# voitta-ai/voitta-rag

Measured on AMD Instinct MI355X. Metric: chunks indexed/sec + p50 top-10 query latency @1M-chunk corpus, 1/8 MI355X, higher is better.
Workload: dtype f16 (f16 MFMA operands, f32 accumulate; softmax, LayerNorm statistics and pooling in f32; the residual stream between layers is stored as f16 (LayerNorm is applied inside the GEMM epilogues from f32 row sums); measured |1-cos| = 1.5e-6 vs the f64 oracle on THIS code path at this scale — 2300 sequenc

## Files before the change

voitta_rag_amd/csrc/prefilter.hip:

```cpp


#include "engine_internal.h"
#include "topk_device.h"

#include <algorithm>
#include <cmath>
#include <vector>

namespace vr {

using f32x4 = __attribute__((ext_vector_type(4))) float;
using f16x8 = __attribute__((ext_vector_type(8))) _Float16;
using half_t = _Float16;

constexpr int kK16 = 32;


__global__ __launch_bounds__(256) void shadow_rows_kernel(const float* __restrict__ corpus, int64_t first_row,
                                                          int64_t n, int dim, int kblocks,
                                                          half_t* __restrict__ corpus16,
                                                          float* __restrict__ row_err) {
  const int lane = threadIdx.x & 63;
  const int64_t row = first_row + static_cast<int64_t>(blockIdx.x) * 4 + (threadIdx.x >> 6);
  if (row >= first_row + n) return;
  const int64_t tile = row / kTileRows;
  const int r = static_cast<int>(row % kTileRows);
  const int kb16n = dim / kK16;
  float e2 = 0.0f;
  for (int k = lane; k < dim; k += 64) {
    const int kb = k / kTileK, kk = k % kTileK;
    const float x = corpus[((tile * kblocks + kb) * 64 + tile_pos(kk % 4, r)) * 4 + kk / 4];
    const float xc = fminf(fmaxf(x, -65504.0f), 65504.0f);
    const half_t h = static_cast<half_t>(xc);
    const float d = x - static_cast<float>(h);
    e2 += d * d;
    const int kb16 = k / kK16, g = (k % kK16) / 8, j = k % 8;
    corpus16[((tile * kb16n + kb16) * 64 + g * 16 + r) * 8 + j] = h;
  }
#pragma unroll
  for (int off = 32; off >= 1; off >>= 1) e2 += __shfl_xor(e2, off);
  if (lane == 0) row_err[row] = sqrtf(e2) * 1.001f + 1.0e-12f;
}

using i32x4 = __attribute__((ext_vector_type(4))) int;
constexpr int kK8 = 64;

__global__ __launch_bounds__(256) void shadow_rows8_kernel(const float* __restrict__ corpus, int64_t first_row,
                                                           int64_t n, int dim, int kblocks,
                                                           int8_t* __restrict__ corpus8,
                                                           float* __restrict__ row_scale,
                                                           float* __restrict__ row_err,
                                                           const float* __restrict__ centre, float centre_norm) {
  const int lane = threadIdx.x & 63;
  const int64_t row = first_row + static_cast<int64_t>(blockIdx.x) * 4 + (threadIdx.x >> 6);
  if (row >= first_row + n) return;
  const int64_t tile = row / kTileRows;
  const int r = static_cast<int>(row % kTileRows);
  const int kb8n = dim / kK8;
  auto at = [&](int k) {
    const int kb = k / kTileK, kk = k % kTileK;
    const float x = corpus[((tile * kblocks + kb) * 64 + tile_pos(kk % 4, r)) * 4 + kk / 4];
    return centre ? x - centre[k] : x;
  };
  float mx = 0.0f;
  for (int k = lane; k < dim; k += 64) mx = fmaxf(mx, fabsf(at(k)));
#pragma unroll
  for (int off = 32; off >= 1; off >>= 1) mx = fmaxf(mx, __shfl_xor(mx, off));
  const bool finite = mx <= 3.0e38f;
  const float s = finite ? mx / 127.0f : 0.0f;
  const float inv = finite && mx > 0.0f ? 127.0f / mx : 0.0f;
  float e2 = 0.0f;
  for (int k = lane; k < dim; k += 64) {
    const float x = at(k);
    const float t = fminf(fmaxf(rintf(x * inv), -127.0f), 127.0f);
    const float d = x - s * t;
    e2 += d * d;
    corpus8[((tile * kb8n + k / kK8) * 64 + ((k % kK8) / 16) * 16 + r) * 16 + k % 16] = static_cast<int8_t>(t);
  }
#pragma unroll
  for (int off = 32; off >= 1; off >>= 1) e2 += __shfl_xor(e2, off);
  if (lane == 0) {
    row_scale[row] = s;
    row_err[row] = finite ? sqrtf(e2) * 1.001f + 2.4e-7f * mx * sqrtf(static_cast<float>(dim)) + 1.0e-12f +
                                (centre ? 1.2e-7f * (1.001f + centre_norm) : 0.0f)
                          : __builtin_inff();
  }
}

int prefilter_store_rows(vr_engine* e, int64_t n, int64_t first_row) {
  if (!e->prefilter || n <= 0) return 0;
  if (e->prefilter8)
    hipLaunchKernelGGL(shadow_rows8_kernel, dim3(static_cast<unsigned>((n + 3) / 4)), dim3(256), 0, e->stream,
                       e->corpus.p, first_row, n, e->dim, e->kblocks, reinterpret_cast<int8_t*>(e->corpus16.p),
                       e->row_scale.p, e->row_err.p, e->centre_rows > 0 ? e->centre.p : static_cast<const float*>(nullptr),
                       e->centre_norm);
  else
    hipLaunchKernelGGL(shadow_rows_kernel, dim3(static_cast<unsigned>((n + 3) / 4)), dim3(256), 0, e->stream,
                       e->corpus.p, first_row, n, e->dim, e->kblocks, reinterpret_cast<half_t*>(e->corpus16.p),
                       e->row_err.p);
  VR_HIP(hipGetLastError());
  return 0;
}

__global__ __launch_bounds__(256) void column_sum_kernel(const float* __restrict__ corpus, int64_t n_rows, int kblocks,
                                                         float* __restrict__ sum) {
  const int64_t tile0 = static_cast<int64_t>(blockIdx.x) * 64;
  const int64_t n_tiles = (n_rows + kTileRows - 1) / kTileRows;
  for (int p = threadIdx.x; p < kblocks * 256; p += 256) {
    const int kb = p >> 8, pos = (p >> 2) & 63, c = p & 3;
    const int r = pos >> 2;
    float acc = 0.0f;
    for (int64_t t = tile0; t < min(tile0 + 64, n_tiles); ++t)
      if (t * kTileRows + r < n_rows) acc += corpus[(t * kblocks + kb) * 256 + p - (kb << 8)];
    atomicAdd(sum + kb * kTileK + (pos & 3) + 4 * c, acc);
  }
}

__global__ void centre_from_sum_kernel(const float* __restrict__ sum, int dim, float inv_n, float* __restrict__ centre) {
  const int k = blockIdx.x * blockDim.x + threadIdx.x;
  if (k < dim) centre[k] = sum[k] * inv_n;
}

constexpr int64_t kCentreMinRows = 1024;

int prefilter_recentre(vr_engine* e) {
  if (!e->prefilter || !e->prefilter8 || e->n_rows <= 0) return 0;
  const bool centring = !(getenv("VR_PREFILTER_CENTRE") && atoi(getenv("VR_PREFILTER_CENTRE")) == 0);
  if (!centring) e->centre_rows = 0;
  e->centre_checked_rows = e->n_rows;
  if (centring && e->n_rows >= kCentreMinRows) {
    static_assert(kTileK == 16, "column_sum_kernel decodes the [k/16][lane][4] image");
    VR_TRY(e->centre.grow(e->dim, 0, e->stream));
    VR_TRY(e->centre_sum.grow(e->dim, 0, e->stream));
    VR_HIP(hipMemsetAsync(e->centre_sum.p, 0, sizeof(float) * static_cast<size_t>(e->dim), e->stream));
    const int64_t n_tiles = (e->n_rows + kTileRows - 1) / kTileRows;
    hipLaunchKernelGGL(column_sum_kernel, dim3(static_cast<unsigned>((n_tiles + 63) / 64)), dim3(256), 0, e->stream,
                       e->corpus.p, e->n_rows, e->kblocks, e->centre_sum.p);
    hipLaunchKernelGGL(centre_from_sum_kernel, dim3(static_cast<unsigned>((e->dim + 255) / 256)), dim3(256), 0, e->stream,
                       e->centre_sum.p, e->dim, 1.0f / static_cast<float>(e->n_rows), e->centre.p);
    VR_HIP(hipGetLastError());
    std::vector<float> host(static_cast<size_t>(e->dim));
    VR_HIP(hipMemcpyAsync(host.data(), e->centre.p, sizeof(float) * host.size(), hipMemcpyDeviceToHost, e->stream));
    VR_HIP(hipStreamSynchronize(e->stream));
    double n2 = 0.0;
    bool finite = true;
    for (float v : host) {
      n2 += static_cast<double>(v) * v;
      finite = finite && std::isfinite(v);
    }
    if (!centring) {
      e->centre_norm = 0.0f;
      e->centre_rows = 0;
    } else if (finite) {
      e->centre_norm = static_cast<float>(std::sqrt(n2) * 1.000001 + 1e-30);
      e->centre_rows = e->n_rows;
    } else {
      e->centre_norm = 0.0f;
      e->centre_rows = 0;
    }
  }
  return prefilter_store_rows(e, e->n_rows, 0);
}


constexpr int kScan16Waves = 8;

__global__ __launch_bounds__(kScan16Waves * 64) void prefilter_scan_kernel(
    const uint4* __restrict__ corpus16, const float* __restrict__ q_img, const float* __restrict__ row_err,
    const uint8_t* __restrict__ mask, int64_t n_tiles, int kb16n, int dim, int k, float* __restrict__ upper,
    uint64_t* __restrict__ cand, int32_t* __restrict__ counter) {
  extern __shared__ uint4 q_lds[];
  __shared__ float red[kScan16Waves];
  uint64_t* lists = reinterpret_cast<uint64_t*>(q_lds + 2 * kb16n * 64);
  if (blockIdx.x == 0 && threadIdx.x == 0) counter[0] = counter[1] = 0;
  for (int i = threadIdx.x; i < 2 * kb16n * 64; i += kScan16Waves * 64) q_lds[i] = make_uint4(0, 0, 0, 0);
  for (int i = threadIdx.x; i < kScan16Waves * kListLen; i += kScan16Waves * 64) lists[i] = 0ull;
  __syncthreads();
  float n2 = 0.0f;
  {
    half_t* qh = reinterpret_cast<half_t*>(q_lds);
    half_t* ql = qh + kb16n * 512;
    for (int kk = threadIdx.x; kk < dim; kk += kScan16Waves * 64) {
      const int kb = kk / kTileK, kr = kk % kTileK;
      const float q = q_img[(kb * 64 + (kr % 4) * 16 + 0) * 4 + kr / 4];
      n2 += q * q;
      const float qc = fminf(fmaxf(q, -65504.0f), 65504.0f);
      const half_t hi = static_cast<half_t>(qc);
      const half_t lo = static_cast<half_t>(qc - static_cast<float>(hi));
      const int at = ((kk / kK16) * 64 + ((kk % kK16) / 8) * 16 + 0) * 8 + kk % 8;
      qh[at] = hi;
      ql[at] = lo;
    }
  }
#pragma unroll
  for (int off = 32; off >= 1; off >>= 1) n2 += __shfl_xor(n2, off);
  if ((threadIdx.x & 63) == 0) red[threadIdx.x >> 6] = n2;
  __syncthreads();
  float qn2 = 0.0f;
#pragma unroll
  for (int w = 0; w < kScan16Waves; ++w) qn2 += red[w];
  const float qn = sqrtf(qn2) * 1.0001f + 1.0e-12f;
  const float c_fixed = 1.001f * (4.8e-7f * qn + 6.0e-8f * sqrtf(static_cast<float>(dim))) +
                        static_cast<float>(dim) * 5.0e-7f * fmaxf(qn, 1.0f);
  const int lane = threadIdx.x & 63;
  const int wave = threadIdx.x >> 6;
  uint64_t* mine = lists + wave * kListLen;
  const bool active = (lane & 15) == 0;
  const int64_t wave_stride = static_cast<int64_t>(gridDim.x) * kScan16Waves;
  for (int64_t tile = static_cast<int64_t>(blockIdx.x) * kScan16Waves + wave; tile < n_tiles; tile += wave_stride) {
    const uint4* src = corpus16 + tile * kb16n * 64 + lane;
    const int64_t row0 = tile * kTileRows + (lane >> 4) * 4;
    uchar4 m = make_uchar4(0, 0, 0, 0);
    float4 e4 = make_float4(0.f, 0.f, 0.f, 0.f);
    if (active) {
      m = *reinterpret_cast<const uchar4*>(mask + row0);
      e4 = *reinterpret_cast<const float4*>(row_err + row0);
    }
    f32x4 acc = {0.0f, 0.0f, 0.0f, 0.0f};
    int kb = 0;
    for (; kb + 8 <= kb16n; kb += 8) {
      uint4 a[8];
#pragma unroll
      for (int u = 0; u < 8; ++u) a[u] = src[(kb + u) * 64];
#pragma unroll
      for (int u = 0; u < 8; ++u) {
        const uint4 bh = q_lds[(kb + u) * 64 + lane];
        const uint4 bl = q_lds[(kb16n + kb + u) * 64 + lane];
        acc = __builtin_amdgcn_mfma_f32_16x16x32_f16(*reinterpret_cast<const f16x8*>(&a[u]),
                                                     *reinterpret_cast<const f16x8*>(&bh), acc, 0, 0, 0);
        acc = __builtin_amdgcn_mfma_f32_16x16x32_f16(*reinterpret_cast<const f16x8*>(&a[u]),
                                                     *reinterpret_cast<const f16x8*>(&bl), acc, 0, 0, 0);
      }
    }
    for (; kb < kb16n; ++kb) {
      const uint4 a = src[kb * 64];
      const uint4 bh = q_lds[kb * 64 + lane];
      const uint4 bl = q_lds[(kb16n + kb) * 64 + lane];
      acc = __builtin_amdgcn_mfma_f32_16x16x32_f16(*reinterpret_cast<const f16x8*>(&a),
                                                   *reinterpret_cast<const f16x8*>(&bh), acc, 0, 0, 0);
      acc = __builtin_amdgcn_mfma_f32_16x16x32_f16(*reinterpret_cast<const f16x8*>(&a),
                                                   *reinterpret_cast<const f16x8*>(&bl), acc, 0, 0, 0);
    }
    uint64_t key[4] = {0, 0, 0, 0};
    if (active) {
      const unsigned char mm[4] = {m.x, m.y, m.z, m.w};
      const float ee[4] = {e4.x, e4.y, e4.z, e4.w};
      float up[4];
#pragma unroll
      for (int r = 0; r < 4; ++r) {
        const float a = acc[r];
        const float err = ee[r] * qn + c_fixed + 2.0e-7f * fabsf(a);
        up[r] = mm[r] ? a + err : -__builtin_inff();
        key[r] = mm[r] ? topk_make_key(a - err, row0 + r) : 0ull;
      }
      *reinterpret_cast<float4*>(upper + row0) = make_float4(up[0], up[1], up[2], up[3]);
    }
    const uint64_t thr = active ? mine[k - 1] : ~0ull;
    if (__ballot(key[0] > thr || key[1] > thr || key[2] > thr || key[3] > thr)) {
#pragma unroll
      for (int r = 0; r < 4; ++r) wave_offer(mine, k, key[r], 0, active, lane);
    }
  }
  block_merge_lists(lists, kListLen, kScan16Waves, wave, lane);
  if (wave == 0) cand[static_cast<int64_t>(blockIdx.x) * kListLen + lane] = lists[lane];
}


__global__ __launch_bounds__(kScan16Waves * 64) void prefilter_scan8_kernel(
    const uint4* __restrict__ corpus8, const float* __restrict__ q_img, const float* __restrict__ row_err,
    const float* __restrict__ row_scale, const uint8_t* __restrict__ mask, int64_t n_tiles, int kb8n, int dim, int k,
    float* __restrict__ upper, uint64_t* __restrict__ cand, int32_t* __restrict__ counter, float centre_norm) {
  extern __shared__ uint4 q_lds[];
  __shared__ float red[3][kScan16Waves];
  uint64_t* lists = reinterpret_cast<uint64_t*>(q_lds + 2 * kb8n * 64);
  if (blockIdx.x == 0 && threadIdx.x == 0) counter[0] = counter[1] = 0;
  for (int i = threadIdx.x; i < 2 * kb8n * 64; i += kScan16Waves * 64) q_lds[i] = make_uint4(0, 0, 0, 0);
  for (int i = threadIdx.x; i < kScan16Waves * kListLen; i += kScan16Waves * 64) lists[i] = 0ull;
  auto q_at = [&](int kk) {
    const int kb = kk / kTileK, kr = kk % kTileK;
    return q_img[(kb * 64 + (kr % 4) * 16 + 0) * 4 + kr / 4];
  };
  float mx = 0.0f, n2 = 0.0f;
  for (int kk = threadIdx.x; kk < dim; kk += kScan16Waves * 64) {
    const float q = q_at(kk);
    mx = fmaxf(mx, fabsf(q));
    n2 += q * q;
  }
#pragma unroll
  for (int off = 32; off >= 1; off >>= 1) {
    mx = fmaxf(mx, __shfl_xor(mx, off));
    n2 += __shfl_xor(n2, off);
  }
  if ((threadIdx.x & 63) == 0) {
    red[0][threadIdx.x >> 6] = mx;
    red[1][threadIdx.x >> 6] = n2;
  }
  __syncthreads();
  float t = 0.0f, qn2 = 0.0f;
#pragma unroll
  for (int w = 0; w < kScan16Waves; ++w) {
    t = fmaxf(t, red[0][w]);
    qn2 += red[1][w];
  }
  const bool q_ok = t > 0.0f && t <= 3.0e38f;
  const float a = q_ok ? t / 127.0f : 0.0f;
  const float inv_a = q_ok ? 127.0f / t : 0.0f;
  const float b = a / 254.0f;
  const float inv_b = a > 0.0f ? 254.0f / a : 0.0f;
  float rho2 = 0.0f;
  {
    int8_t* qa = reinterpret_cast<int8_t*>(q_lds);
    int8_t* qb = qa + kb8n * 1024;
    for (int kk = threadIdx.x; kk < dim; kk += kScan16Waves * 64) {
      const float q = q_at(kk);
      const float ta = fminf(fmaxf(rintf(q * inv_a), -127.0f), 127.0f);
      const float r = q - a * ta;
      const float tb = fminf(fmaxf(rintf(r * inv_b), -127.0f), 127.0f);
      const float rho = r - b * tb;
      rho2 += rho * rho;
      const int at = ((kk / kK8) * 64 + ((kk % kK8) / 16) * 16 + 0) * 16 + kk % 16;
      qa[at] = static_cast<int8_t>(ta);
      qb[at] = static_cast<int8_t>(tb);
    }
  }
#pragma unroll
  for (int off = 32; off >= 1; off >>= 1) rho2 += __shfl_xor(rho2, off);
  if ((threadIdx.x & 63) == 0) red[2][threadIdx.x >> 6] = rho2;
  __syncthreads();
  float rho2_all = 0.0f;
#pragma unroll
  for (int w = 0; w < kScan16Waves; ++w) rho2_all += red[2][w];
  const float qn = sqrtf(qn2) * 1.0001f + 1.0e-12f;
  const float rho_n = q_ok ? sqrtf(rho2_all) * 1.001f + 3.0e-7f * qn + 1.0e-12f : __builtin_inff();
  const float c_fixed = static_cast<float>(dim) * 5.0e-7f * fmaxf(qn, 1.0f) + 1.0e-7f * qn * sqrtf(static_cast<float>(dim)) +
                        centre_norm * rho_n;
  const int lane = threadIdx.x & 63;
  const int wave = threadIdx.x >> 6;
  uint64_t* mine = lists + wave * kListLen;
  const bool active = (lane & 15) == 0;
  const int64_t wave_stride = static_cast<int64_t>(gridDim.x) * kScan16Waves;
  for (int64_t tile = static_cast<int64_t>(blockIdx.x) * kScan16Waves + wave; tile < n_tiles; tile += wave_stride) {
    const uint4* src = corpus8 + tile * kb8n * 64 + lane;
    const int64_t row0 = tile * kTileRows + (lane >> 4) * 4;
    uchar4 m = make_uchar4(0, 0, 0, 0);
    float4 e4 = make_float4(0.f, 0.f, 0.f, 0.f), s4 = e4;
    if (active) {
      m = *reinterpret_cast<const uchar4*>(mask + row0);
      e4 = *reinterpret_cast<const float4*>(row_err + row0);
      s4 = *reinterpret_cast<const float4*>(row_scale + row0);
    }
    i32x4 acc_a = {0, 0, 0, 0}, acc_b = {0, 0, 0, 0};
    int kb = 0;
    for (; kb + 6 <= kb8n; kb += 6) {
      uint4 v[6];
#pragma unroll
      for (int u = 0; u < 6; ++u) v[u] = src[(kb + u) * 64];
#pragma unroll
      for (int u = 0; u < 6; ++u) {
        const uint4 ba = q_lds[(kb + u) * 64 + lane];
        const uint4 bb = q_lds[(kb8n + kb + u) * 64 + lane];
        acc_a = __builtin_amdgcn_mfma_i32_16x16x64_i8(*reinterpret_cast<const i32x4*>(&v[u]),
                                                      *reinterpret_cast<const i32x4*>(&ba), acc_a, 0, 0, 0);
        acc_b = __builtin_amdgcn_mfma_i32_16x16x64_i8(*reinterpret_cast<const i32x4*>(&v[u]),
                                                      *reinterpret_cast<const i32x4*>(&bb), acc_b, 0, 0, 0);
      }
    }
    for (; kb < kb8n; ++kb) {
      const uint4 v = src[kb * 64];
      const uint4 ba = q_lds[kb * 64 + lane];
      const uint4 bb = q_lds[(kb8n + kb) * 64 + lane];
      acc_a = __builtin_amdgcn_mfma_i32_16x16x64_i8(*reinterpret_cast<const i32x4*>(&v),
                                                    *reinterpret_cast<const i32x4*>(&ba), acc_a, 0, 0, 0);
      acc_b = __builtin_amdgcn_mfma_i32_16x16x64_i8(*reinterpret_cast<const i32x4*>(&v),
                                                    *reinterpret_cast<const i32x4*>(&bb), acc_b, 0, 0, 0);
    }
    uint64_t key[4] = {0, 0, 0, 0};
    if (active) {
      const unsigned char mm[4] = {m.x, m.y, m.z, m.w};
      const float ee[4] = {e4.x, e4.y, e4.z, e4.w};
      const float ss[4] = {s4.x, s4.y, s4.z, s4.w};
      float up[4];
#pragma unroll
      for (int r = 0; r < 4; ++r) {
        const float fa = a * static_cast<float>(acc_a[r]);
        const float fb = b * static_cast<float>(acc_b[r]);
        const float score = ss[r] * (fa + fb);
        const float err = ee[r] * qn + (1.001f + ee[r]) * rho_n + c_fixed + 2.0e-6f * ss[r] * (fabsf(fa) + fabsf(fb));
        up[r] = mm[r] ? score + err : -__builtin_inff();
        key[r] = mm[r] ? topk_make_key(score - err, row0 + r) : 0ull;
      }
      *reinterpret_cast<float4*>(upper + row0) = make_float4(up[0], up[1], up[2], up[3]);
    }
    const uint64_t thr = active ? mine[k - 1] : ~0ull;
    if (__ballot(key[0] > thr || key[1] > thr || key[2] > thr || key[3] > thr)) {
#pragma unroll
      for (int r = 0; r < 4; ++r) wave_offer(mine, k, key[r], 0, active, lane);
    }
  }
  block_merge_lists(lists, kListLen, kScan16Waves, wave, lane);
  if (wave == 0) cand[static_cast<int64_t>(blockIdx.x) * kListLen + lane] = lists[lane];
}


__device__ __forceinline__ float key_score(uint64_t key) {
  const uint32_t hi = static_cast<uint32_t>(key >> 32);
  const uint32_t u = (hi & 0x80000000u) ? (hi ^ 0x80000000u) : ~hi;
  return __uint_as_float(u);
}

__global__ __launch_bounds__(256) void collect_candidates_kernel(const float* __restrict__ upper, int64_t n,
                                                                 const uint64_t* __restrict__ lower_keys, int k,
                                                                 int32_t* __restrict__ tiles,
                                                                 int32_t* __restrict__ masks, int32_t* counter) {
  const uint64_t kth = lower_keys[k - 1];
  const float thr = kth ? key_score(kth) : -3.0e38f;
  const int lane = threadIdx.x & 63;
  const int64_t base = (static_cast<int64_t>(blockIdx.x) * blockDim.x + threadIdx.x) * 4;
  float4 u = make_float4(-__builtin_inff(), -__builtin_inff(), -__builtin_inff(), -__builtin_inff());
  if (base < n) u = *reinterpret_cast<const float4*>(upper + base);
  const float uu[4] = {u.x, u.y, u.z, u.w};
  int m = 0;
#pragma unroll
  for (int c = 0; c < 4; ++c)
    if (base + c < n && uu[c] >= thr) m |= 1 << c;
  if (__ballot(m != 0) == 0) return;
  int m16 = m << (4 * (lane & 3));
  m16 |= __shfl_xor(m16, 1);
  m16 |= __shfl_xor(m16, 2);
  const bool take = (lane & 3) == 0 && m16 != 0;
  const uint64_t takers = __ballot(take);
  int rows_here = take ? __popc(m16) : 0;
#pragma unroll
  for (int off = 32; off >= 1; off >>= 1) rows_here += __shfl_xor(rows_here, off);
  const int leader = __builtin_ctzll(takers);
  int slot0 = 0;
  if (lane == leader) {
    slot0 = atomicAdd(counter, __popcll(takers));
    atomicAdd(counter + 1, rows_here);
  }
  slot0 = __shfl(slot0, leader);
  const int slot = slot0 + __popcll(takers & ((1ull << lane) - 1ull));
  if (take && slot < kMaxCandTiles) {
    tiles[slot] = static_cast<int32_t>(base / kTileRows);
    masks[slot] = m16;
  }
}


constexpr int kRescoreThreads = 1024;
constexpr int kRescoreBlocks = 128;
constexpr int kRescoreChunk = 64;

__global__ __launch_bounds__(kRescoreThreads) void rescore_kernel(const float4* __restrict__ corpus,
                                                                  const float4* __restrict__ q_img, int kblocks,
                                                                  const int32_t* __restrict__ tiles,
                                                                  const int32_t* __restrict__ masks,
                                                                  const int32_t* __restrict__ counter, int k,
                                                                  uint64_t* __restrict__ lists_out,
                                                                  int32_t* __restrict__ out_count) {
  extern __shared__ float4 stage[];
  __shared__ uint64_t best[kListLen];
  const int chunk = min(kblocks, kRescoreChunk);
  const bool q_resident = kblocks <= kRescoreChunk;
  const int n_tiles = counter[0];
  const int count = min(n_tiles, kMaxCandTiles);
  const int lane = threadIdx.x & 63;
  const int wave = threadIdx.x >> 6;
  if (blockIdx.x == 0 && threadIdx.x == 0) *out_count = n_tiles > kMaxCandTiles ? 0x7fffffff : counter[1];
  if (threadIdx.x < kListLen) best[threadIdx.x] = 0ull;
  bool q_staged = !q_resident;
  const bool active = (lane & 15) == 0;
  for (int c = blockIdx.x; c < count; c += gridDim.x) {
    const int64_t tile = tiles[c];
    const int mask = masks[c];
    f32x4 acc = {0.0f, 0.0f, 0.0f, 0.0f};
    for (int kb0 = 0; kb0 < kblocks; kb0 += chunk) {
      const int nkb = min(chunk, kblocks - kb0);
      const float4* a_src = corpus + (tile * kblocks + kb0) * 64;
      const float4* b_src = q_img + kb0 * 64;
      __syncthreads();
#pragma unroll 4
      for (int i = threadIdx.x; i < nkb * 64; i += kRescoreThreads) {
        stage[i] = a_src[i];
        if (!q_staged || !q_resident) stage[chunk * 64 + i] = b_src[i];
      }
      q_staged = true;
      __syncthreads();
      if (wave == 0) {
#pragma unroll 4
        for (int kb = 0; kb < nkb; ++kb) {
          const float4 a = stage[kb * 64 + tile_pos(lane >> 4, lane & 15)];
          const float4 b = stage[(chunk + kb) * 64 + lane];
          acc = __builtin_amdgcn_mfma_f32_16x16x4f32(a.x, b.x, acc, 0, 0, 0);
          acc = __builtin_amdgcn_mfma_f32_16x16x4f32(a.y, b.y, acc, 0, 0, 0);
          acc = __builtin_amdgcn_mfma_f32_16x16x4f32(a.z, b.z, acc, 0, 0, 0);
          acc = __builtin_amdgcn_mfma_f32_16x16x4f32(a.w, b.w, acc, 0, 0, 0);
        }
      }
    }
    if (wave == 0) {
      const int r0 = (lane >> 4) * 4;
#pragma unroll
      for (int r = 0; r < 4; ++r) {
        const uint64_t key = active && ((mask >> (r0 + r)) & 1) ? topk_make_key(acc[r], tile * kTileRows + r0 + r) : 0ull;
        wave_offer(best, k, key, 0, active, lane);
      }
    }
  }
  __syncthreads();
  if (wave == 0) lists_out[static_cast<int64_t>(blockIdx.x) * kListLen + lane] = best[lane];
}

bool prefilter_usable(vr_engine* e, int nq, int k) {
  return e->prefilter && nq == 1 && k <= kFusedMaxK && e->n_rows >= 4096;
}

int prefilter_search(vr_engine* e, int k, const uint8_t* mask_dev, uint64_t* out_keys_dev, int32_t* out_count_dev) {
  const int kb16n = e->dim / kK16;
  const int64_t n_tiles = (e->n_rows + kTileRows - 1) / kTileRows;
  VR_TRY(e->upper.grow(e->cap_rows, 0, e->stream));
  VR_TRY(e->cand_rows.grow(2 * kMaxCandTiles + 16, 0, e->stream));
  int64_t blocks = std::min<int64_t>((n_tiles + kScan16Waves - 1) / kScan16Waves, kScanBlocks);
  VR_TRY(e->cand_a.grow(std::max<int64_t>(blocks, kRescoreBlocks) * kListLen, 0, e->stream));
  VR_TRY(e->cand_b.grow(kListLen, 0, e->stream));
  int32_t* counter = e->cand_rows.p + 2 * kMaxCandTiles;
  hipStream_t s = e->stream;
  if (e->prefilter8) {
    const int kb8n = e->dim / kK8;
    const size_t lds = static_cast<size_t>(2) * kb8n * 1024 + kScan16Waves * kListLen * sizeof(uint64_t);
    if (lds > 64 * 1024)
      VR_HIP(hipFuncSetAttribute(reinterpret_cast<const void*>(prefilter_scan8_kernel),
                                 hipFuncAttributeMaxDynamicSharedMemorySize, static_cast<int>(lds)));
    prof_begin(e, VR_PROF_DENSE_SCAN, static_cast<double>(e->n_rows) * (e->dim * 1.0 + 4.0 + 4.0 + 1.0 + 4.0));
    hipLaunchKernelGGL(prefilter_scan8_kernel, dim3(static_cast<unsigned>(blocks)), dim3(kScan16Waves * 64), lds, s,
                       reinterpret_cast<const uint4*>(e->corpus16.p), e->q_tiled.p, e->row_err.p, e->row_scale.p,
                       mask_dev, n_tiles, kb8n, e->dim, k, e->upper.p, e->cand_a.p, counter,
                       e->centre_rows > 0 ? e->centre_norm : 0.0f);
    prof_end(e);
  } else {
    const size_t lds = static_cast<size_t>(2) * kb16n * 1024 + kScan16Waves * kListLen * sizeof(uint64_t);
    if (lds > 64 * 1024)
      VR_HIP(hipFuncSetAttribute(reinterpret_cast<const void*>(prefilter_scan_kernel),
                                 hipFuncAttributeMaxDynamicSharedMemorySize, static_cast<int>(lds)));
    prof_begin(e, VR_PROF_DENSE_SCAN, static_cast<double>(e->n_rows) * (e->dim * 2.0 + 4.0 + 1.0 + 4.0));
    hipLaunchKernelGGL(prefilter_scan_kernel, dim3(static_cast<unsigned>(blocks)), dim3(kScan16Waves * 64), lds, s,
                       reinterpret_cast<const uint4*>(e->corpus16.p), e->q_tiled.p, e->row_err.p, mask_dev, n_tiles,
                       kb16n, e->dim, k, e->upper.p, e->cand_a.p, counter);
    prof_end(e);
  }
  VR_TRY(topk_merge_lists(e, e->cand_a.p, static_cast<int>(blocks), 1, k, e->cand_b.p));
  const int64_t n4 = (e->n_rows + 3) / 4;
  int32_t* cand_tiles = e->cand_rows.p;
  int32_t* cand_masks = e->cand_rows.p + kMaxCandTiles;
  hipLaunchKernelGGL(collect_candidates_kernel, dim3(static_cast<unsigned>((n4 + 255) / 256)), dim3(256), 0, s,
                     e->upper.p, e->n_rows, e->cand_b.p, k, cand_tiles, cand_masks, counter);
  const size_t rescore_lds = static_cast<size_t>(2) * std::min(e->kblocks, kRescoreChunk) * 1024;
  if (rescore_lds > 64 * 1024)
    VR_HIP(hipFuncSetAttribute(reinterpret_cast<const void*>(rescore_kernel),
                               hipFuncAttributeMaxDynamicSharedMemorySize, static_cast<int>(rescore_lds)));
  hipLaunchKernelGGL(rescore_kernel, dim3(kRescoreBlocks), dim3(kRescoreThreads), rescore_lds, s,
                     reinterpret_cast<const float4*>(e->corpus.p),
                     reinterpret_cast<const float4*>(e->q_tiled.p), e->kblocks, cand_tiles, cand_masks, counter, k,
                     e->cand_a.p, out_count_dev);
  VR_TRY(topk_merge_lists(e, e->cand_a.p, kRescoreBlocks, 1, k, out_keys_dev));
  VR_HIP(hipGetLastError());
  return 0;
}

}
```

voitta_rag_amd/csrc/topk.hip:

```cpp

#include "engine_internal.h"
#include "topk_device.h"

namespace vr {

__device__ __forceinline__ uint64_t make_key(float s, int64_t row) {
  if (s == -__builtin_inff()) return 0ull;
  uint32_t u = __float_as_uint(s);
  u = (u & 0x80000000u) ? ~u : (u | 0x80000000u);
  return (static_cast<uint64_t>(u) << 32) | static_cast<uint32_t>(0xFFFFFFFFu - static_cast<uint32_t>(row));
}

template <int THREADS, int ITEMS>
__device__ __forceinline__ void block_extract_topk(uint64_t (&keys)[ITEMS], int k,
                                                   uint64_t* __restrict__ out) {
  constexpr int WAVES = THREADS / 64;
  __shared__ uint64_t wmax[2][WAVES];
  const int lane = threadIdx.x & 63;
  const int wave = threadIdx.x >> 6;

  uint64_t lmax = 0;
#pragma unroll
  for (int i = 0; i < ITEMS; ++i) lmax = keys[i] > lmax ? keys[i] : lmax;

  for (int r = 0; r < k; ++r) {
    uint64_t m = lmax;
#pragma unroll
    for (int off = 32; off >= 1; off >>= 1) {
      uint64_t o = __shfl_xor(m, off);
      m = o > m ? o : m;
    }
    if (lane == 0) wmax[r & 1][wave] = m;
    __syncthreads();
    uint64_t best = 0;
#pragma unroll
    for (int w = 0; w < WAVES; ++w) {
      uint64_t v = wmax[r & 1][w];
      best = v > best ? v : best;
    }
    if (threadIdx.x == 0) out[r] = best;
    if (best == 0) {
      for (int j = r + 1 + threadIdx.x; j < k; j += THREADS) out[j] = 0;
      break;
    }
    if (lmax == best) {
      lmax = 0;
#pragma unroll
      for (int i = 0; i < ITEMS; ++i) {
        if (keys[i] == best) keys[i] = 0;
        lmax = keys[i] > lmax ? keys[i] : lmax;
      }
    }
  }
}

template <int THREADS, int ITEMS>
__global__ __launch_bounds__(THREADS) void select_from_scores_kernel(
    const float* __restrict__ scores, int64_t stride, int64_t n, int k, uint64_t* __restrict__ out) {
  const int64_t seg = blockIdx.x;
  const int q = blockIdx.y;
  const int64_t base = seg * (THREADS * ITEMS);
  const float* s = scores + q * stride;
  uint64_t keys[ITEMS];
#pragma unroll
  for (int i = 0; i < ITEMS; ++i) {
    int64_t row = base + i * THREADS + threadIdx.x;
    keys[i] = row < n ? make_key(s[row], row) : 0ull;
  }
  block_extract_topk<THREADS, ITEMS>(keys, k, out + (static_cast<int64_t>(q) * gridDim.x + seg) * k);
}

template <int THREADS, int ITEMS>
__global__ __launch_bounds__(THREADS) void select_from_keys_kernel(const uint64_t* __restrict__ in,
                                                                   int64_t count, int k,
                                                                   uint64_t* __restrict__ out) {
  const int64_t seg = blockIdx.x;
  const int q = blockIdx.y;
  const int64_t base = seg * (THREADS * ITEMS);
  const uint64_t* s = in + q * count;
  uint64_t keys[ITEMS];
#pragma unroll
  for (int i = 0; i < ITEMS; ++i) {
    int64_t j = base + i * THREADS + threadIdx.x;
    keys[i] = j < count ? s[j] : 0ull;
  }
  block_extract_topk<THREADS, ITEMS>(keys, k, out + (static_cast<int64_t>(q) * gridDim.x + seg) * k);
}

template <int THREADS, int ITEMS>
__global__ __launch_bounds__(THREADS) void select_regions_kernel(const uint64_t* __restrict__ in, int n_reg, int cap,
                                                                 const int32_t* __restrict__ cnt,
                                                                 const uint64_t* __restrict__ spill, int spill_cap,
                                                                 const int32_t* __restrict__ spill_cnt, int k,
                                                                 uint64_t* __restrict__ out,
                                                                 int32_t* __restrict__ overflow,
                                                                 int32_t* __restrict__ total_out,
                                                                 int32_t* __restrict__ overflow_q) {
  __shared__ uint64_t gat[THREADS * ITEMS];
  __shared__ int n_gat;
  const int q = blockIdx.x;
  const int n_spill = spill_cnt ? spill_cnt[q] : 0;
  if (threadIdx.x == 0) n_gat = n_spill < spill_cap ? n_spill : spill_cap;
  __syncthreads();
  for (int j = threadIdx.x; j < n_spill && j < spill_cap; j += THREADS)
    if (j < THREADS * ITEMS) gat[j] = spill[static_cast<int64_t>(q) * spill_cap + j];
  const uint64_t* base = in + static_cast<int64_t>(q) * n_reg * cap;
  const int32_t* c = cnt + static_cast<int64_t>(q) * n_reg;
  for (int r = threadIdx.x; r < n_reg; r += THREADS) {
    const int have = c[r];
    if (have <= 0) continue;
    const int n = have < cap ? have : cap;
    const int at = atomicAdd(&n_gat, n);
    for (int j = 0; j < n; ++j)
      if (at + j < THREADS * ITEMS) gat[at + j] = base[static_cast<int64_t>(r) * cap + j];
  }
  __syncthreads();
  const int total = n_gat;
  if (threadIdx.x == 0) {
    if (total_out) atomicAdd(total_out, total);
    if (n_spill > spill_cap || total > THREADS * ITEMS) {
      *overflow = 1;
      if (overflow_q) overflow_q[q] = 1;
    }
  }
  uint64_t keys[ITEMS];
#pragma unroll
  for (int i = 0; i < ITEMS; ++i) {
    const int j = i * THREADS + static_cast<int>(threadIdx.x);
    keys[i] = j < total && j < THREADS * ITEMS ? gat[j] : 0ull;
  }
  block_extract_topk<THREADS, ITEMS>(keys, k, out + static_cast<int64_t>(q) * k);
}

int topk_select_regions(vr_engine* e, const uint64_t* cand, int n_reg, int cap, const int32_t* cnt, const uint64_t* spill,
                        int spill_cap, const int32_t* spill_cnt, int nq, int k, uint64_t* out, int32_t* overflow_mapped,
                        int32_t* total_dev, int32_t* overflow_q) {
  VR_CHECK(k >= 1 && k <= kMaxK && nq >= 1 && cap >= 1 && n_reg >= 1, "bad region-select shape");
  hipLaunchKernelGGL((select_regions_kernel<1024, 8>), dim3(static_cast<unsigned>(nq)), dim3(1024), 0, e->stream, cand, n_reg, cap,
                     cnt, spill, spill_cap, spill_cnt, k, out, overflow_mapped, total_dev, overflow_q);
  VR_HIP(hipGetLastError());
  return 0;
}


constexpr int kMergeThreads = 1024;
constexpr int kMergeWaves = kMergeThreads / 64;
constexpr int kMergeMaxLists = 512;
constexpr int kGatherCap = 2048;
constexpr int kGatherBatch = 16;

__global__ __launch_bounds__(kMergeThreads) void merge_lists_kernel(uint64_t* __restrict__ cand, int n_lists,
                                                                     int k, uint64_t* __restrict__ out) {
  __shared__ uint64_t gat[kGatherCap];
  __shared__ uint64_t wave_thr[kMergeWaves];
  __shared__ uint64_t heads[kMergeMaxLists];
  __shared__ uint64_t head_thr;
  __shared__ int gathered;
  const int lane = threadIdx.x & 63;
  const int wave = threadIdx.x >> 6;
  uint64_t* in = cand + static_cast<int64_t>(blockIdx.x) * n_lists * kListLen;
  uint64_t* dst = out + static_cast<int64_t>(blockIdx.x) * k;

  {
    uint64_t t = 0;
    if (static_cast<int>(threadIdx.x) < n_lists) {
      heads[threadIdx.x] = in[threadIdx.x * kListLen];
      t = in[threadIdx.x * kListLen + (k - 1)];
    }
#pragma unroll
    for (int off = 32; off >= 1; off >>= 1) {
      const uint64_t o = __shfl_xor(t, off);
      t = o > t ? o : t;
    }
    if (lane == 0) wave_thr[wave] = t;
    if (threadIdx.x == 0) {
      gathered = 0;
      head_thr = 0;
    }
    __syncthreads();
    if (static_cast<int>(threadIdx.x) < n_lists) {
      const uint64_t h = heads[threadIdx.x];
      int rank = 0;
      for (int j = 0; j < n_lists; ++j) rank += heads[j] > h;
      if (rank == k - 1 && h != 0) head_thr = h;
    }
    __syncthreads();
    uint64_t thr = head_thr;
#pragma unroll
    for (int w = 0; w < kMergeWaves; ++w) thr = wave_thr[w] > thr ? wave_thr[w] : thr;
    for (int l0 = wave; l0 < n_lists; l0 += kMergeWaves * kGatherBatch) {
      uint64_t keys[kGatherBatch];
#pragma unroll
      for (int u = 0; u < kGatherBatch; ++u) {
        const int l = min(l0 + u * kMergeWaves, n_lists - 1);
        keys[u] = in[l * kListLen + lane];
      }
#pragma unroll
      for (int u = 0; u < kGatherBatch; ++u) {
        const uint64_t key = keys[u];
        const bool take = l0 + u * kMergeWaves < n_lists && lane < k && key != 0 && key >= thr;
        const uint64_t m = __ballot(take);
        if (m) {
          int base = 0;
          if (lane == 0) base = atomicAdd(&gathered, __popcll(m));
          base = __builtin_amdgcn_readfirstlane(base);
          const int slot = base + __popcll(m & ((1ull << lane) - 1ull));
          if (take && slot < kGatherCap) gat[slot] = key;
        }
      }
    }
    __syncthreads();
    const int c = gathered;
    if (c <= kGatherCap) {
      for (int i = threadIdx.x; i < c; i += kMergeThreads) {
        const uint64_t key = gat[i];
        int rank = 0;
        for (int j = 0; j < c; ++j) rank += gat[j] > key;
        if (rank < k) dst[rank] = key;
      }
      for (int i = c + threadIdx.x; i < k; i += kMergeThreads) dst[i] = 0;
      return;
    }
  }
  int n = n_lists;
  while (n > 1) {
    const int pairs = (n + 1) / 2;
    for (int p0 = 0; p0 < pairs; p0 += kMergeWaves) {
      const int p = p0 + wave;
      uint64_t res = 0;
      if (p < pairs) {
        const uint64_t a = in[(2 * p) * kListLen + lane];
        const uint64_t b = (2 * p + 1 < n) ? in[(2 * p + 1) * kListLen + (63 - lane)] : 0ull;
        res = merge64(a, b, lane);
      }
      __syncthreads();
      if (p < pairs) in[p * kListLen + lane] = res;
    }
    __syncthreads();
    n = pairs;
  }
  if (wave == 0 && lane < k) dst[lane] = in[lane];
}

int topk_merge_lists(vr_engine* e, uint64_t* cand, int n_lists, int nq, int k, uint64_t* out) {
  VR_CHECK(k >= 1 && k <= kListLen && n_lists >= 1 && n_lists <= kMergeMaxLists, "bad merge shape");
  hipLaunchKernelGGL(merge_lists_kernel, dim3(static_cast<unsigned>(nq)), dim3(kMergeThreads), 0, e->stream,
                     cand, n_lists, k, out);
  VR_HIP(hipGetLastError());
  return 0;
}

constexpr int kPartsMax = 4096;

__global__ __launch_bounds__(256) void merge_parts_kernel(const uint64_t* __restrict__ parts, int n_parts, int n_lists,
                                                          int k, int64_t* __restrict__ gid, float* __restrict__ score,
                                                          int32_t* __restrict__ cnt) {
  __shared__ uint64_t keys[kPartsMax];
  __shared__ int total;
  const int l = blockIdx.x;
  const int n = n_parts * k;
  if (threadIdx.x == 0) total = 0;
  for (int i = threadIdx.x; i < n; i += 256) {
    const int p = i / k, j = i - p * k;
    keys[i] = parts[(static_cast<int64_t>(p) * n_lists + l) * k + j];
  }
  for (int j = threadIdx.x; j < k; j += 256) {
    gid[static_cast<int64_t>(l) * k + j] = -1;
    score[static_cast<int64_t>(l) * k + j] = 0.0f;
  }
  __syncthreads();
  int mine = 0;
  for (int i = threadIdx.x; i < n; i += 256) {
    const uint64_t key = keys[i];
    if (key == 0) continue;
    ++mine;
    int rank = 0;
    for (int o = 0; o < n; ++o) {
      const uint64_t ok = keys[o];
      rank += (ok > key) || (ok == key && o < i);
    }
    if (rank < k) {
      const uint32_t hi = static_cast<uint32_t>(key >> 32);
      const uint32_t u = (hi & 0x80000000u) ? (hi ^ 0x80000000u) : ~hi;
      const int64_t row = static_cast<int64_t>(0xFFFFFFFFu - static_cast<uint32_t>(key & 0xFFFFFFFFu));
      gid[static_cast<int64_t>(l) * k + rank] = row * n_parts + i / k;
      score[static_cast<int64_t>(l) * k + rank] = __uint_as_float(u);
    }
  }
  if (mine) atomicAdd(&total, mine);
  __syncthreads();
  if (threadIdx.x == 0) cnt[l] = total < k ? total : k;
}

int topk_merge_parts(vr_engine* e, const uint64_t* parts_dev, int n_parts, int n_lists, int k, int64_t* gid_dev,
                     float* score_dev, int32_t* cnt_dev) {
  VR_CHECK(n_parts >= 1 && n_lists >= 1 && k >= 1 && n_parts * k <= kPartsMax, "merge of %d parts x %d keys (at most %d keys per list)",
           n_parts, k, kPartsMax);
  hipLaunchKernelGGL(merge_parts_kernel, dim3(static_cast<unsigned>(n_lists)), dim3(256), 0, e->stream, parts_dev, n_parts,
                     n_lists, k, gid_dev, score_dev, cnt_dev);
  VR_HIP(hipGetLastError());
  return 0;
}

int topk_select(vr_engine* e, const float* scores, int64_t stride, int64_t n, int nq, int k,
                const uint64_t** out_keys) {
  VR_CHECK(k >= 1 && k <= kMaxK, "top-k of %d not in 1..%d", k, kMaxK);
  VR_CHECK(nq >= 1, "no queries");
  constexpr int T1 = 256, I1 = kTopkSeg / T1;
  constexpr int T2 = 1024, I2 = 16;
  int64_t nseg = (n + kTopkSeg - 1) / kTopkSeg;
  if (nseg < 1) nseg = 1;
  int64_t need = static_cast<int64_t>(nq) * nseg * k;
  VR_TRY(e->cand_a.grow(need, 0, e->stream));
  VR_TRY(e->cand_b.grow(need, 0, e->stream));
  hipLaunchKernelGGL((select_from_scores_kernel<T1, I1>), dim3(static_cast<unsigned>(nseg), nq),
                     dim3(T1), 0, e->stream, scores, stride, n, k, e->cand_a.p);
  uint64_t* cur = e->cand_a.p;
  uint64_t* nxt = e->cand_b.p;
  int64_t count = nseg * k;
  while (nseg > 1) {
    int64_t nseg2 = (count + T2 * I2 - 1) / (T2 * I2);
    hipLaunchKernelGGL((select_from_keys_kernel<T2, I2>), dim3(static_cast<unsigned>(nseg2), nq),
                       dim3(T2), 0, e->stream, cur, count, k, nxt);
    uint64_t* t = cur;
    cur = nxt;
    nxt = t;
    nseg = nseg2;
    count = nseg * k;
  }
  VR_HIP(hipGetLastError());
  *out_keys = cur;
  return 0;
}

}
```

voitta_rag_amd/csrc/topk_device.h:

```cpp
#pragma once

#include <hip/hip_runtime.h>

#include <cstdint>

namespace vr {

constexpr int kListLen = 64;

__device__ __forceinline__ uint64_t topk_make_key(float s, int64_t row) {
  if (s == -__builtin_inff()) return 0ull;
  uint32_t u = __float_as_uint(s);
  u = (u & 0x80000000u) ? ~u : (u | 0x80000000u);
  return (static_cast<uint64_t>(u) << 32) |
         static_cast<uint32_t>(0xFFFFFFFFu - static_cast<uint32_t>(row));
}

__device__ __forceinline__ uint64_t readlane_u64(uint64_t v, int src_lane) {
  uint32_t lo = __builtin_amdgcn_readlane(static_cast<uint32_t>(v), src_lane);
  uint32_t hi = __builtin_amdgcn_readlane(static_cast<uint32_t>(v >> 32), src_lane);
  return (static_cast<uint64_t>(hi) << 32) | lo;
}

__device__ __forceinline__ void wave_list_insert(uint64_t* list, int k, uint64_t key, int lane) {
  const uint64_t cur = list[lane];
  const uint64_t greater = __ballot(cur > key);
  const int pos = __popcll(greater);
  if (pos >= k) return;
  const uint64_t prev = __shfl_up(cur, 1);
  if (lane == pos) list[lane] = key;
  else if (lane > pos && lane < k) list[lane] = prev;
}

__device__ __forceinline__ void wave_offer(uint64_t* lists, int k, uint64_t key, int q_of_lane,
                                           bool active, int lane) {
  uint64_t thr = active ? lists[q_of_lane * kListLen + (k - 1)] : ~0ull;
  uint64_t pending = __ballot(active && key > thr);
  while (pending) {
    const int src = __builtin_ctzll(pending);
    const uint64_t kk = readlane_u64(key, src);
    const int qs = __builtin_amdgcn_readlane(q_of_lane, src);
    wave_list_insert(lists + qs * kListLen, k, kk, lane);
    pending &= pending - 1;
  }
}

__device__ __forceinline__ uint64_t merge64(uint64_t a, uint64_t b_reversed, int lane) {
  uint64_t v = a > b_reversed ? a : b_reversed;
#pragma unroll
  for (int d = 32; d >= 1; d >>= 1) {
    const uint64_t p = __shfl_xor(v, d);
    const bool keep_max = (lane & d) == 0;
    v = keep_max ? (v > p ? v : p) : (v < p ? v : p);
  }
  return v;
}

__device__ __forceinline__ void block_merge_lists(uint64_t* lists, int stride, int n_waves, int wave, int lane) {
  for (int s = 1; s < n_waves; s <<= 1) {
    __syncthreads();
    uint64_t merged = 0;
    const bool mine = (wave % (2 * s)) == 0;
    if (mine) merged = merge64(lists[wave * stride + lane], lists[(wave + s) * stride + (63 - lane)], lane);
    __syncthreads();
    if (mine) lists[wave * stride + lane] = merged;
  }
  __syncthreads();
}

}
```

Baseline: 46880.

## Fold list-merge threshold into candidate collection and rescore two tiles per block

```diff
diff --git a/voitta_rag_amd/csrc/prefilter.hip b/voitta_rag_amd/csrc/prefilter.hip
--- a/voitta_rag_amd/csrc/prefilter.hip
+++ b/voitta_rag_amd/csrc/prefilter.hip
@@ -408,11 +408,19 @@
   return __uint_as_float(u);
 }
 
-__global__ __launch_bounds__(256) void collect_candidates_kernel(const float* __restrict__ upper, int64_t n,
-                                                                 const uint64_t* __restrict__ lower_keys, int k,
-                                                                 int32_t* __restrict__ tiles,
-                                                                 int32_t* __restrict__ masks, int32_t* counter) {
-  const uint64_t kth = lower_keys[k - 1];
+constexpr int kCollectThreads = 1024;
+static_assert(kCollectThreads >= kScanBlocks, "lists_kth_lower_bound: a thread per list");
+
+__global__ __launch_bounds__(kCollectThreads) void collect_candidates_kernel(const float* __restrict__ upper, int64_t n,
+                                                                             const uint64_t* __restrict__ lists,
+                                                                             int n_lists, int k,
+                                                                             int32_t* __restrict__ tiles,
+                                                                             int32_t* __restrict__ masks,
+                                                                             int32_t* counter) {
+  __shared__ uint64_t heads[kScanBlocks];
+  __shared__ uint64_t wave_thr[kCollectThreads / 64];
+  __shared__ uint64_t head_thr;
+  const uint64_t kth = lists_kth_lower_bound(lists, n_lists, k, heads, wave_thr, &head_thr);
   const float thr = kth ? key_score(kth) : -3.0e38f;
   const int lane = threadIdx.x & 63;
   const int64_t base = (static_cast<int64_t>(blockIdx.x) * blockDim.x + threadIdx.x) * 4;
@@ -449,7 +457,9 @@
 
 constexpr int kRescoreThreads = 1024;
 constexpr int kRescoreBlocks = 128;
-constexpr int kRescoreChunk = 64;
+constexpr int kRescoreTiles = 2;
+constexpr int kRescoreChunk = 48;
+static_assert(kRescoreBlocks * kRescoreTiles <= kMaxCandTiles, "a block reads its first slots before it knows the tile count");
 
 __global__ __launch_bounds__(kRescoreThreads) void rescore_kernel(const float4* __restrict__ corpus,
                                                                   const float4* __restrict__ q_img, int kblocks,
@@ -459,38 +469,51 @@
                                                                   uint64_t* __restrict__ lists_out,
                                                                   int32_t* __restrict__ out_count) {
   extern __shared__ float4 stage[];
-  __shared__ uint64_t best[kListLen];
+  __shared__ uint64_t best[kRescoreTiles][kListLen];
   const int chunk = min(kblocks, kRescoreChunk);
-  const bool q_resident = kblocks <= kRescoreChunk;
+  float4* q_b = stage + kRescoreTiles * chunk * 64;
+  const int lane = threadIdx.x & 63;
+  const int wave = threadIdx.x >> 6;
+  const int blocks = static_cast<int>(gridDim.x);
+  int64_t tile0 = tiles[blockIdx.x], tile1 = tiles[blockIdx.x + blocks];
   const int n_tiles = counter[0];
   const int count = min(n_tiles, kMaxCandTiles);
-  const int lane = threadIdx.x & 63;
-  const int wave = threadIdx.x >> 6;
   if (blockIdx.x == 0 && threadIdx.x == 0) *out_count = n_tiles > kMaxCandTiles ? 0x7fffffff : counter[1];
-  if (threadIdx.x < kListLen) best[threadIdx.x] = 0ull;
-  bool q_staged = !q_resident;
+  if (threadIdx.x < kRescoreTiles * kListLen) (&best[0][0])[threadIdx.x] = 0ull;
+  for (int i = threadIdx.x; i < kblocks * 4; i += kRescoreThreads) q_b[i] = q_img[(i >> 2) * 64 + (i & 3) * 16];
   const bool active = (lane & 15) == 0;
-  for (int c = blockIdx.x; c < count; c += gridDim.x) {
-    const int64_t tile = tiles[c];
-    const int mask = masks[c];
+  for (int c0 = blockIdx.x; c0 < count; c0 += blocks * kRescoreTiles) {
+    const bool two = c0 + blocks < count;
+    if (c0 != static_cast<int>(blockIdx.x)) {
+      tile0 = tiles[c0];
+      tile1 = two ? tiles[c0 + blocks] : 0;
+    }
+    const int mine = c0 + wave * blocks;
+    const bool chains = wave < kRescoreTiles && mine < count;
+    const int mask = chains ? masks[mine] : 0;
     f32x4 acc = {0.0f, 0.0f, 0.0f, 0.0f};
     for (int kb0 = 0; kb0 < kblocks; kb0 += chunk) {
       const int nkb = min(chunk, kblocks - kb0);
-      const float4* a_src = corpus + (tile * kblocks + kb0) * 64;
-      const float4* b_src = q_img + kb0 * 64;
       __syncthreads();
-#pragma unroll 4
+      const float4* src0 = corpus + (tile0 * kblocks + kb0) * 64;
+      const float4* src1 = corpus + (tile1 * kblocks + kb0) * 64;
+#pragma unroll 2
       for (int i = threadIdx.x; i < nkb * 64; i += kRescoreThreads) {
-        stage[i] = a_src[i];
-        if (!q_staged || !q_resident) stage[chunk * 64 + i] = b_src[i];
-      }
-      q_staged = true;
+        const float4 v0 = src0[i];
+        if (two) {
+          const float4 v1 = src1[i];
+          stage[chunk * 64 + i] = v1;
+        }
+        stage[i] = v0;
+      }
       __syncthreads();
-      if (wave == 0) {
+      if (chains) {
+        const float4* a_lds = stage + wave * chunk * 64 + tile_pos(lane >> 4, lane & 15);
+        const float4* b_lds = q_b + kb0 * 4 + (lane >> 4);
 #pragma unroll 4
         for (int kb = 0; kb < nkb; ++kb) {
-          const float4 a = stage[kb * 64 + tile_pos(lane >> 4, lane & 15)];
-          const float4 b = stage[(chunk + kb) * 64 + lane];
+          const float4 a = a_lds[kb * 64];
+          const float4 b = b_lds[kb * 4];
           acc = __builtin_amdgcn_mfma_f32_16x16x4f32(a.x, b.x, acc, 0, 0, 0);
           acc = __builtin_amdgcn_mfma_f32_16x16x4f32(a.y, b.y, acc, 0, 0, 0);
           acc = __builtin_amdgcn_mfma_f32_16x16x4f32(a.z, b.z, acc, 0, 0, 0);
@@ -498,17 +521,20 @@
         }
       }
     }
-    if (wave == 0) {
+    if (chains) {
+      const int64_t tile = wave == 0 ? tile0 : tile1;
       const int r0 = (lane >> 4) * 4;
 #pragma unroll
       for (int r = 0; r < 4; ++r) {
         const uint64_t key = active && ((mask >> (r0 + r)) & 1) ? topk_make_key(acc[r], tile * kTileRows + r0 + r) : 0ull;
-        wave_offer(best, k, key, 0, active, lane);
+        wave_offer(best[wave], k, key, 0, active, lane);
       }
     }
   }
   __syncthreads();
-  if (wave == 0) lists_out[static_cast<int64_t>(blockIdx.x) * kListLen + lane] = best[lane];
+  static_assert(kRescoreTiles == 2, "two tile images are staged, two lists folded by one merge64");
+  if (wave == 0)
+    lists_out[static_cast<int64_t>(blockIdx.x) * kListLen + lane] = merge64(best[0][lane], best[1][63 - lane], lane);
 }
 
 bool prefilter_usable(vr_engine* e, int nq, int k) {
@@ -522,7 +548,6 @@
   VR_TRY(e->cand_rows.grow(2 * kMaxCandTiles + 16, 0, e->stream));
   int64_t blocks = std::min<int64_t>((n_tiles + kScan16Waves - 1) / kScan16Waves, kScanBlocks);
   VR_TRY(e->cand_a.grow(std::max<int64_t>(blocks, kRescoreBlocks) * kListLen, 0, e->stream));
-  VR_TRY(e->cand_b.grow(kListLen, 0, e->stream));
   int32_t* counter = e->cand_rows.p + 2 * kMaxCandTiles;
   hipStream_t s = e->stream;
   if (e->prefilter8) {
@@ -548,13 +573,14 @@
                        kb16n, e->dim, k, e->upper.p, e->cand_a.p, counter);
     prof_end(e);
   }
-  VR_TRY(topk_merge_lists(e, e->cand_a.p, static_cast<int>(blocks), 1, k, e->cand_b.p));
   const int64_t n4 = (e->n_rows + 3) / 4;
   int32_t* cand_tiles = e->cand_rows.p;
   int32_t* cand_masks = e->cand_rows.p + kMaxCandTiles;
-  hipLaunchKernelGGL(collect_candidates_kernel, dim3(static_cast<unsigned>((n4 + 255) / 256)), dim3(256), 0, s,
-                     e->upper.p, e->n_rows, e->cand_b.p, k, cand_tiles, cand_masks, counter);
-  const size_t rescore_lds = static_cast<size_t>(2) * std::min(e->kblocks, kRescoreChunk) * 1024;
+  hipLaunchKernelGGL(collect_candidates_kernel, dim3(static_cast<unsigned>((n4 + kCollectThreads - 1) / kCollectThreads)),
+                     dim3(kCollectThreads), 0, s, e->upper.p, e->n_rows, e->cand_a.p, static_cast<int>(blocks), k, cand_tiles,
+                     cand_masks, counter);
+  const size_t rescore_lds = static_cast<size_t>(kRescoreTiles) * std::min(e->kblocks, kRescoreChunk) * 1024 +
+                             static_cast<size_t>(e->kblocks) * 4 * sizeof(float4);
   if (rescore_lds > 64 * 1024)
     VR_HIP(hipFuncSetAttribute(reinterpret_cast<const void*>(rescore_kernel),
                                hipFuncAttributeMaxDynamicSharedMemorySize, static_cast<int>(rescore_lds)));
diff --git a/voitta_rag_amd/csrc/topk.hip b/voitta_rag_amd/csrc/topk.hip
--- a/voitta_rag_amd/csrc/topk.hip
+++ b/voitta_rag_amd/csrc/topk.hip
@@ -162,32 +162,8 @@
   uint64_t* dst = out + static_cast<int64_t>(blockIdx.x) * k;
 
   {
-    uint64_t t = 0;
-    if (static_cast<int>(threadIdx.x) < n_lists) {
-      heads[threadIdx.x] = in[threadIdx.x * kListLen];
-      t = in[threadIdx.x * kListLen + (k - 1)];
-    }
-#pragma unroll
-    for (int off = 32; off >= 1; off >>= 1) {
-      const uint64_t o = __shfl_xor(t, off);
-      t = o > t ? o : t;
-    }
-    if (lane == 0) wave_thr[wave] = t;
-    if (threadIdx.x == 0) {
-      gathered = 0;
-      head_thr = 0;
-    }
-    __syncthreads();
-    if (static_cast<int>(threadIdx.x) < n_lists) {
-      const uint64_t h = heads[threadIdx.x];
-      int rank = 0;
-      for (int j = 0; j < n_lists; ++j) rank += heads[j] > h;
-      if (rank == k - 1 && h != 0) head_thr = h;
-    }
-    __syncthreads();
-    uint64_t thr = head_thr;
-#pragma unroll
-    for (int w = 0; w < kMergeWaves; ++w) thr = wave_thr[w] > thr ? wave_thr[w] : thr;
+    if (threadIdx.x == 0) gathered = 0;
+    const uint64_t thr = lists_kth_lower_bound(in, n_lists, k, heads, wave_thr, &head_thr);
     for (int l0 = wave; l0 < n_lists; l0 += kMergeWaves * kGatherBatch) {
       uint64_t keys[kGatherBatch];
 #pragma unroll
diff --git a/voitta_rag_amd/csrc/topk_device.h b/voitta_rag_amd/csrc/topk_device.h
--- a/voitta_rag_amd/csrc/topk_device.h
+++ b/voitta_rag_amd/csrc/topk_device.h
@@ -68,4 +68,32 @@
   __syncthreads();
 }
 
+__device__ __forceinline__ uint64_t lists_kth_lower_bound(const uint64_t* __restrict__ in, int n_lists, int k,
+                                                          uint64_t* heads, uint64_t* wave_thr, uint64_t* head_thr) {
+  const int lane = threadIdx.x & 63;
+  uint64_t t = 0;
+  if (static_cast<int>(threadIdx.x) < n_lists) {
+    heads[threadIdx.x] = in[threadIdx.x * kListLen];
+    t = in[threadIdx.x * kListLen + (k - 1)];
+  }
+#pragma unroll
+  for (int off = 32; off >= 1; off >>= 1) {
+    const uint64_t o = __shfl_xor(t, off);
+    t = o > t ? o : t;
+  }
+  if (lane == 0) wave_thr[threadIdx.x >> 6] = t;
+  if (threadIdx.x == 0) *head_thr = 0;
+  __syncthreads();
+  if (static_cast<int>(threadIdx.x) < n_lists) {
+    const uint64_t h = heads[threadIdx.x];
+    int rank = 0;
+    for (int j = 0; j < n_lists; ++j) rank += heads[j] > h;
+    if (rank == k - 1 && h != 0) *head_thr = h;
+  }
+  __syncthreads();
+  uint64_t thr = *head_thr;
+  for (int w = 0; w < static_cast<int>(blockDim.x >> 6); ++w) thr = wave_thr[w] > thr ? wave_thr[w] : thr;
+  return thr;
 }
+
+}
```

Result: no change. 47030, median of 5 (+0.3%).
